# slatedb/slatedb

Hardware: AMD Instinct MI355X
Metric: GiB/s device-resident SST block encode+bloom, 64 MiB sorted KV, 1/2/4/8 GPU (higher is better)
Workload: dtype u8

## Files before the change

slatedb_amd/csrc/sdb_encode.h:

```cpp
#pragma once
#include <hip/hip_runtime.h>
#include <stdint.h>

#include "../../include/slatedb_amd.h"
#include "sdb_workspace.h"

namespace sdb {

constexpr uint32_t kChunk = 2048;
constexpr uint32_t kResolveLds = 96 * 1024;
#ifndef SDB_EMIT_CRC_MFMA
#define SDB_EMIT_CRC_SLICE
#endif
#ifdef SDB_EMIT_CRC_SLICE
constexpr uint32_t kCrcLds = 36 * 1024;
#else
constexpr uint32_t kCrcLds = 56 * 1024;
#endif
constexpr uint32_t kImgCap = 4096 + 64;
constexpr uint32_t kStageCap = 4096;
constexpr uint32_t kStageGuard = 64;
constexpr uint32_t kKeyStageCap = 1024;
constexpr uint32_t kPieceRowMax = 4000, kPieceKeyMax = 960, kPieceValMax = 3968;
constexpr uint32_t kSegLook = 1024;
constexpr uint32_t kSegSpan = kChunk + kSegLook;
constexpr uint32_t kSegThreads = 512;
constexpr uint32_t kFactsThreads = 1024;
constexpr uint32_t kFactsPerT = 2;
constexpr uint32_t kFactsEntries = kFactsThreads * kFactsPerT;
constexpr uint32_t kSegLds = (2 * kSegSpan + 4) * 4 + kChunk * 6;
constexpr uint32_t kSegLdsMax = 64 * 1024;
constexpr uint32_t kHashPerT = kChunk / kSegThreads;
#ifndef SDB_EMIT_WAVES
#define SDB_EMIT_WAVES 16
#endif
constexpr uint32_t kEmitThreads = 64 * SDB_EMIT_WAVES;
constexpr uint32_t kEmitWgPerCu = 1;
constexpr uint32_t kEmitWaveLds = kStageGuard + kImgCap + 16 + kKeyStageCap + 64 * 16;
constexpr uint32_t kEmitLds = kCrcLds + 16 + (kEmitThreads / 64) * kEmitWaveLds;
constexpr uint32_t kEnumLds = kChunk * 16 + 11 * kChunk * 2;
constexpr uint32_t kEnumTabLds = 11 * kChunk * 2;
constexpr uint32_t kGroupThreads = 1024;
constexpr uint32_t kEnumThreads = 512;
constexpr uint32_t kGroupLds = kResolveLds;

struct BloomPlan {
    uint32_t k, m;
    uint32_t sb;
    uint32_t nslices, T, tiles;
    uint32_t one_pass;
    uint32_t pad;
    uint64_t mmod;
};
struct BloomSlots {
    uint32_t *count;
    uint32_t *slot;
    uint32_t cap;
};

struct BlockDesc {
    uint32_t s, e;
    uint64_t off;
    uint64_t vs, ve, ks, ke;
    uint32_t bb, pad;
};

struct EncodeArgs {
    const uint8_t *key_bytes;
    const uint64_t *key_off;
    const uint8_t *val_bytes;
    const uint64_t *val_off;
    const uint8_t *kind;
    const uint64_t *seq;
    const int64_t *create_ts;
    const int64_t *expire_ts;
    const uint8_t *ts_mask;
    uint64_t n;
    uint32_t block_size;
    uint32_t restart_interval;
    uint32_t version;
    uint32_t wal;
    uint32_t nchunks;
    uint32_t seg_look;
    uint32_t *lcp;
    uint32_t *szr, *sznr;
    uint32_t nfacts;
    uint32_t *row_scratch;
    uint32_t *next;
    uint32_t *bbytes;
    uint32_t *tab_exit;
    uint32_t *tab_cnt;
    uint64_t *tab_bytes;
    uint32_t *anchor_e;
    uint32_t *anchor_blk;
    uint64_t *anchor_byte;
    unsigned long long *err;
    uint32_t *wmax;
    uint32_t *slow_count;
    uint32_t *slow_list;
    uint32_t *big_count;
    uint32_t *big_list;
    BlockDesc *desc;
    uint64_t *stat_part;
    uint32_t *huge_part;
    uint32_t *wmax_part;
    unsigned long long *err_part;
    uint32_t *gtab_exit;
    uint32_t *gtab_cnt;
    uint64_t *gtab_bytes;
    uint32_t *mode;
    uint32_t group;
    uint32_t bloom_fused;
    BloomPlan bpl;
    BloomSlots bq;
    uint8_t *bloom_out;
    uint32_t *done;
    uint32_t nprep_wg;
    uint32_t seg_lds;
    uint8_t *out_data;
    uint64_t *out_block_off;
    uint32_t *out_block_first;
    uint32_t *out_index_key_len;
// ... 175 lines not shown
```

slatedb_amd/csrc/sdb_encode.hip:

```cpp
#include <stdlib.h>

#include <atomic>
#include <mutex>

#include "sdb_bloom.h"
#include "sdb_crc.h"
#include "sdb_crc_mfma.h"

namespace sdb {

#ifndef SDB_SEG_WAVES
#define SDB_SEG_WAVES 8
#endif
#ifdef SDB_PHASE_TIMING
__device__ uint64_t g_phase[1024][8];
#define PHASE_MARK(i)                                                              \
    do {                                                                           \
        __syncthreads();                                                           \
        if (threadIdx.x == 0 && blockIdx.x < 1024) g_phase[blockIdx.x][i] = __builtin_amdgcn_s_memtime(); \
    } while (0)
__device__ uint64_t g_wave_phase[8192][8];
__device__ uint64_t g_phase_enum[1024][8];
#define PHASE_MARK_E(i)                                                                  \
    do {                                                                                 \
// ... 274 lines not shown
#ifdef SDB_EXP_FACTS_NOBIN
        bloom_bin_core<kFactsPerT>(blockIdx.x, hh, dd, 0, a.bpl, a.bq, blds);
#else
        bloom_bin_core<kFactsPerT>(blockIdx.x, hh, dd, nk, a.bpl, a.bq, blds);
#endif
    }
}

SDB_DEV uint32_t walk_size_v2(const EncodeArgs &a, uint64_t j, bool rs) {
    EntryFacts f = entry_facts(a, j);
    return rs ? f.s_r : f.s_nr;
}

SDB_DEV void seg_chunk(const EncodeArgs &a, uint8_t *smem, uint32_t k) {
    uint32_t *s_P = (uint32_t *)smem;
    uint32_t *s_R = s_P + kSegSpan + 4;
    uint32_t *s_bb = s_R + kSegSpan;
    uint16_t *s_nx = (uint16_t *)(s_bb + kChunk);
    __shared__ uint32_t s_len[kSegThreads / 64];
    const uint32_t tid = threadIdx.x, nt = blockDim.x;
    const uint64_t cs = (uint64_t)k * kChunk;
    const uint64_t ce = cs + kChunk < a.n ? cs + kChunk : a.n;
    const uint64_t se = ce + a.seg_look < a.n ? ce + a.seg_look : a.n;
    const uint32_t cn = (uint32_t)(ce - cs), sn = (uint32_t)(se - cs);
    const uint64_t bs = a.block_size;
    const uint32_t clampv = (uint32_t)(bs + 16);
    const bool v2 = a.version == 2 && bs <= (1u << 20);
    const uint32_t ri = a.restart_interval;
    PHASE_MARK(0);
    constexpr uint32_t kPerT = kSegSpan / kSegThreads;
    const uint32_t lane = (uint32_t)lane_id();
    uint32_t zr[kPerT], znr[kPerT];
#pragma unroll
    for (uint32_t u = 0; u < kPerT; u++) {
        const uint32_t x = tid + u * nt;
        zr[u] = znr[u] = 0;
        if (x < sn) {
            zr[u] = a.szr[cs + x];
            znr[u] = a.sznr[cs + x];
        }
    }
#pragma unroll
    for (uint32_t u = 0; u < kPerT; u++) {
        const uint32_t x = tid + u * nt;
        if (x >= sn) continue;
        if (v2) {
            const uint32_t cr = zr[u] < clampv ? zr[u] : clampv, cnr = znr[u] < clampv ? znr[u] : clampv;
            s_P[x] = cnr;
            s_R[x] = cr + 2 - cnr;
        }
    }
    __syncthreads();
    PHASE_MARK(1);
    if (v2) {
        __shared__ uint32_t s_wt[kPerT * (kSegThreads / 64) + 1];
        const uint32_t wv = tid >> 6;
        uint32_t v[kPerT], inc[kPerT];
#pragma unroll
        for (uint32_t u = 0; u < kPerT; u++) {
            const uint32_t x = tid + u * nt;
            v[u] = x < sn ? s_P[x] : 0;
            inc[u] = wave_incl_scan(v[u]);
            if (lane == 63) s_wt[u * (nt >> 6) + wv] = inc[u];
        }
        __syncthreads();
        if (tid < 64) {
            const uint32_t nw = kPerT * (nt >> 6);
            const uint32_t t = tid < nw ? s_wt[tid] : 0, it = wave_incl_scan(t);
            __builtin_amdgcn_wave_barrier();
            if (tid < nw) s_wt[tid] = it - t;
            if (tid == 63) s_P[sn] = it;
        }
        __syncthreads();
#pragma unroll
        for (uint32_t u = 0; u < kPerT; u++) {
            const uint32_t x = tid + u * nt;
            if (x < sn) s_P[x] = s_wt[u * (nt >> 6) + wv] + inc[u] - v[u];
        }
        PHASE_MARK(2);
    }
    __syncthreads();
    PHASE_MARK(3);
    uint32_t maxlen = 0;
    for (uint32_t x = tid; x < cn; x += nt) {
        const uint64_t b = cs + x;
        uint64_t j;
        uint64_t bytes;
        if (v2) {
            const uint32_t Pb = s_P[x];
            auto size_of = [&](uint32_t e) -> uint64_t {
                uint64_t sz = 2ull + (s_P[e] - Pb);
                for (uint32_t r = x; r < e; r += ri) sz += s_R[r];
                return sz;
            };
            uint32_t lo = x + 1;
            uint32_t e = lo;
            {
                const uint32_t w = (x + 64 < sn ? x + 64 : sn) - x;
                const uint32_t mean = (s_P[x + w] - Pb) / w + 1;
                uint32_t est = x + (uint32_t)(bs / mean);
                e = est < lo ? lo : (est > sn ? sn : est);
            }
            if (size_of(e) <= bs) {
                while (e < sn && size_of(e + 1) <= bs) e++;
            } else {
                while (e > lo && size_of(e) > bs) e--;
            }
            j = cs + e;
            if (e == lo) bytes = 2ull + a.szr[b] + 2;
            else bytes = size_of(e);
            if (e == sn && se < a.n) {
                uint64_t acc = bytes;
                uint32_t p = e - x, ph = p % ri;
                while (j < a.n) {
                    const bool rs = ph == 0;
                    const uint64_t add = (uint64_t)walk_size_v2(a, j, rs) + (rs ? 2 : 0);
                    if (acc + add > bs) break;
                    acc += add;
                    j++;
                    if (++ph == ri) ph = 0;
                }
                bytes = acc;
            }
        } else if (a.version == 2) {
            uint64_t acc = 2;
            j = b;
            uint32_t p = 0, ph = 0;
            while (j < a.n) {
                const bool rs = ph == 0;
                const uint64_t add = (uint64_t)walk_size_v2(a, j, rs) + (rs ? 2 : 0);
                if (p > 0 && acc + add > bs) break;
                acc += add;
                j++;
                p++;
                if (++ph == ri) ph = 0;
            }
            bytes = acc;
        } else {
            uint64_t acc = 2;
            j = b;
            uint32_t p = 0;
            const uint64_t fko = a.key_off[b];
            const uint32_t fkl = (uint32_t)(a.key_off[b + 1] - fko);
            while (j < a.n) {
                uint32_t prefix = 0;
                if (p > 0) {
                    uint64_t ko = a.key_off[j];
                    prefix = lcp_bytes(a.key_bytes + fko, fkl, a.key_bytes + ko, (uint32_t)(a.key_off[j + 1] - ko));
                }
                uint64_t sr = a.szr[j];
                uint64_t sz = sr - prefix;
                if (p > 0 && acc + sz > bs) break;
                acc += sz + 2;
                j++;
                p++;
            }
            bytes = acc;
        }
        const uint32_t bb = (uint32_t)(bytes + 4);
        a.next[b] = (uint32_t)j;
        a.bbytes[b] = bb;
        s_bb[x] = bb;
        const uint64_t rel = j - cs;
        s_nx[x] = (uint16_t)(rel < 0xFFFF ? rel : 0xFFFF);
        const uint32_t len = (uint32_t)(j - b);
        maxlen = len > maxlen ? len : maxlen;
    }
    maxlen = wave_max(maxlen);
    if (lane_id() == 0) s_len[tid >> 6] = maxlen;
    __syncthreads();
    if (tid == 0) {
        uint32_t m = 0;
        for (uint32_t q = 0; q < nt / 64; q++) m = s_len[q] > m ? s_len[q] : m;
        a.wmax_part[k] = m;
    }
    PHASE_MARK(4);
    __shared__ uint32_t s_wc;
    if (tid == 0) {
        uint32_t wc = a.seg_look;
        if (v2) {
            uint32_t lo = 0, hi = sn;
            while (lo < hi) {
                const uint32_t mid = (lo + hi + 1) >> 1;
                if ((uint64_t)(s_P[mid] - s_P[0]) + 2 <= bs) lo = mid;
                else hi = mid - 1;
            }
            wc = lo + 1 < wc ? lo + 1 : wc;
        }
        s_wc = wc;
    }
    __syncthreads();
    const uint32_t Wc = s_wc;
    uint32_t *j_nx = s_P;
    uint64_t *j_bb = (uint64_t *)(s_P + kChunk);
    static_assert(3 * kChunk <= 2 * kSegSpan + 4, "jump tables alias s_P / s_R");
    constexpr uint32_t kJU = kChunk / kSegThreads;
    {
        uint32_t jn[kJU];
        uint64_t jb[kJU];
#pragma unroll
        for (uint32_t u = 0; u < kJU; u++) {
            const uint32_t x = tid + u * nt;
            jn[u] = 0;
            jb[u] = 0;
            if (x < cn) {
                const uint32_t n1 = s_nx[x];
                uint64_t b = s_bb[x];
                uint32_t n = n1, c = 1;
                if (n1 < cn) {
                    b += s_bb[n1];
                    n = s_nx[n1];
                    c = 2;
                }
                jn[u] = n | c << 16;
                jb[u] = b;
            }
        }
#pragma unroll
        for (uint32_t u = 0; u < kJU; u++) {
            const uint32_t x = tid + u * nt;
            if (x < cn) {
                j_nx[x] = jn[u];
                j_bb[x] = jb[u];
            }
        }
        __syncthreads();
#pragma unroll
        for (uint32_t u = 0; u < kJU; u++) {
            const uint32_t x = tid + u * nt;
            if (x < cn) {
                const uint32_t n = jn[u] & 0xFFFF;
                if (n < cn) {
                    const uint32_t w = j_nx[n];
                    jb[u] += j_bb[n];
                    jn[u] = (w & 0xFFFF) | ((jn[u] >> 16) + (w >> 16)) << 16;
                }
            }
        }
        __syncthreads();
#pragma unroll
        for (uint32_t u = 0; u < kJU; u++) {
            const uint32_t x = tid + u * nt;
            if (x < cn) {
                j_nx[x] = jn[u];
                j_bb[x] = jb[u];
            }
        }
        __syncthreads();
    }
    for (uint32_t c = tid; c < Wc; c += nt) {
        uint32_t e = c, cnt = 0;
        uint64_t by = 0;
        while (e < cn) {
            const uint32_t v = j_nx[e];
            by += j_bb[e];
            cnt += v >> 16;
            e = v & 0xFFFF;
        }
        const uint64_t t = (uint64_t)k * a.seg_look + c;
        a.tab_exit[t] = c >= cn ? (uint32_t)ce : (e == 0xFFFF ? 0xFFFFFFFFu : (uint32_t)(cs + e));
        a.tab_cnt[t] = cnt;
        a.tab_bytes[t] = by;
    }
    PHASE_MARK(5);
    PHASE_MARK(6);
}

__global__ __launch_bounds__(kSegThreads, SDB_SEG_WAVES) void k_seg(SstSet P) {
    const EncodeArgs a = make_args(P, blockIdx.y);
    extern __shared__ __attribute__((aligned(16))) uint8_t smem[];
    if (blockIdx.x < P.max_chunks) {
        if (blockIdx.x < a.nchunks) seg_chunk(a, smem, blockIdx.x);
    } else if (a.bloom_fused && blockIdx.x - P.max_chunks < a.bpl.nslices) {
        bloom_fill_slice(blockIdx.x - P.max_chunks, a.key_bytes, a.key_off, a.n, a.bpl, a.bq, a.bloom_out,
                         a.bloom_len, (uint32_t *)smem);
    }
}

__global__ __launch_bounds__(kGroupThreads) void k_group(SstSet P) {
// ... 1555 lines not shown
            } else {
                q = (int)(r + l);
            }
            if (q >= 0) {
                if (tr_lds) {
                    tr[2 * q] = (uint8_t)(br >> 8);
                    tr[2 * q + 1] = (uint8_t)br;
                } else {
                    gblk[D + 2 * q] = (uint8_t)(br >> 8);
                    gblk[D + 2 * q + 1] = (uint8_t)br;
                }
            }
        }
        wave_sync();
        if (l < 16) ((lu32 *)(img - kStageGuard))[l] = 0;
        if (r == 0 && l == 0) ((lu32 *)img)[0] = ~((const lu32 *)img)[0];
        wave_sync();
        crc = crc_shift_bytes(crc, Lp) ^ wave_crc_image_ra(img, Lp) ^ 0xFFFFFFFFu;
        uint8_t *gp = gblk + base;
        const uint32_t nfull = Lp >> 4;
        for (uint32_t cc = l; cc < nfull; cc += 64) {
            u32x4 v = ((const lu128 *)img)[cc];
            if (cc == 0 && r == 0) v.x = ~v.x;
            __builtin_memcpy(gp + 16 * cc, &v, 16);
        }
        if (l < (Lp & 15)) {
            const uint32_t x = (nfull << 4) + l;
            gp[x] = (r == 0 && x < 4) ? (uint8_t)~img[x] : img[x];
        }
        pu += (uint32_t)__popcll(__ballot(prow && kind == SDB_KIND_VALUE));
        de += (uint32_t)__popcll(__ballot(prow && kind == SDB_KIND_TOMBSTONE));
        me += (uint32_t)__popcll(__ballot(prow && kind == SDB_KIND_MERGE));
        base += Lp;
        r += c;
        wave_sync();
    }
    if (base != D && l == 0) report_error(a.err, d.s, SDB_DEVICE_ERROR);
    if (tr_lds) {
        if (l == 0) {
            tr[2 * noffs] = (uint8_t)(noffs >> 8);
            tr[2 * noffs + 1] = (uint8_t)noffs;
        }
        wave_sync();
        const uint8_t v = l < Tl ? tr[l] : 0;
        if (l < 16) ((lu32 *)(img - kStageGuard))[l] = 0;
        img[l] = v;
        wave_sync();
        crc = crc_shift_bytes(crc, Tl) ^ wave_crc_image_ra(img, Tl) ^ 0xFFFFFFFFu;
        if (l < Tl) gblk[D + l] = v;
    } else {
        if (l == 0) {
            gblk[D + 2 * noffs] = (uint8_t)(noffs >> 8);
            gblk[D + 2 * noffs + 1] = (uint8_t)noffs;
        }
        __threadfence_block();
        wave_sync();
    }
    for (uint32_t t = tr_lds ? Lc : D; t < Lc; t += 4096) {
        const uint32_t w = Lc - t < 4096 ? Lc - t : 4096;
        for (uint32_t q = l; q < w; q += 64) img[q] = gblk[t + q];
        if (l < 16) ((lu32 *)(img - kStageGuard))[l] = 0;
        for (uint32_t q = w + l; q < ((w + 63) & ~63u); q += 64) img[q] = 0;
        wave_sync();
        crc = crc_shift_bytes(crc, w) ^ wave_crc_image_ra(img, w) ^ 0xFFFFFFFFu;
        wave_sync();
    }
    crc ^= 0xFFFFFFFFu;
    if (l == 0) {
        gblk[Lc] = (uint8_t)(crc >> 24);
        gblk[Lc + 1] = (uint8_t)(crc >> 16);
        gblk[Lc + 2] = (uint8_t)(crc >> 8);
        gblk[Lc + 3] = (uint8_t)crc;
        a.out_block_stats[3 * (uint64_t)blk] = (uint16_t)pu;
        a.out_block_stats[3 * (uint64_t)blk + 1] = (uint16_t)de;
        a.out_block_stats[3 * (uint64_t)blk + 2] = (uint16_t)me;
        a.out_index_key_len[blk] = ik;
    }
    wave_sync();
}

template <int V>
SDB_DEV void emit_slow_blocks(const EncodeArgs &a, uint8_t *scratch, const uint32_t (*s_crc)[256]);

SDB_DEV void finish_summary(const EncodeArgs &a) {
    sdb_sst_summary *s = a.summary;
    const unsigned long long e = atomicOr(a.err, 0ull);
    s->max_block_entries = *a.wmax;
    uint64_t bl = a.bloom_len;
    if (a.bloom_len_dev) {
        bl = *a.bloom_len_dev;
        if (bl == ~0ull) {
            bl = 0;
            if (e == ~0ull) {
                s->status = SDB_INVALID_ARGUMENT;
                s->first_error_entry = 0;
            }
        }
    }
    s->bloom_len = bl;
    s->num_probes = a.num_probes;
    s->filter_built = a.filter_built;
    if (e != ~0ull) {
        s->status = (int32_t)(e & 0xFF);
        s->first_error_entry = e >> 8;
    }
}

template <int V>
__global__ __launch_bounds__(kEmitThreads, 1) void k_emit(SstSet P) {
    extern __shared__ __attribute__((aligned(16))) uint8_t smem[];
#ifdef SDB_PHASE_TIMING
    const uint64_t rt0 = __builtin_amdgcn_s_memrealtime(), mt0 = __builtin_amdgcn_s_memtime();
#endif
    const uint32_t wave = (uint32_t)__builtin_amdgcn_readfirstlane((int)(threadIdx.x >> 6)), wpb = blockDim.x >> 6;
    const uint32_t gw = blockIdx.x * wpb + wave;
    (void)gw;
    const uint32_t l = (uint32_t)lane_id();
    uint64_t ph[8] = {0, 0, 0, 0, 0, 0, 0, 0};
    uint32_t nbl = 0;
    if (l < P.count) {
        const EncodeArgs ai = make_args(P, l);
        if (*ai.err == ~0ull) nbl = ai.anchor_blk[ai.nchunks];
    }
    const uint32_t vpre = wave_incl_scan(nbl);
    const uint32_t nb = (uint32_t)__builtin_amdgcn_readlane((int)vpre, kMaxSsts - 1);
    bool run = nb > 0;
    if (lds_addr((const void *)smem) != 0) {
        if (threadIdx.x == 0)
            for (uint32_t i = 0; i < P.count; i++) report_error(make_args(P, i).err, 0, SDB_DEVICE_ERROR);
        run = false;
    }
    auto locate = [&](uint32_t g, uint32_t &si, uint32_t &lb) {
        const uint64_t m = __ballot(l + 1 < kMaxSsts && vpre <= g && vpre < nb);
        si = (uint32_t)__popcll(m);
        lb = g - (si ? (uint32_t)__builtin_amdgcn_readlane((int)vpre, (int)si - 1) : 0u);
    };
    auto desc_lanes = [&](uint32_t g, uint32_t r1) -> uint32_t {
        uint32_t si, lb;
        locate(g < r1 ? g : r1 - 1, si, lb);
        return ((const uint32_t *)make_args(P, si).desc)[14 * (uint64_t)lb + (l < 14 ? l : 13)];
    };
    if (run) {
        lu32 *crc = (lu32 *)smem;
        (void)crc;
        const uint32_t r0 = (uint32_t)((uint64_t)nb * blockIdx.x / gridDim.x);
        const uint32_t r1 = (uint32_t)((uint64_t)nb * (blockIdx.x + 1) / gridDim.x);
        uint32_t blk = r0 + wave;
        const bool any = blk < r1;
        uint32_t dvc = any ? desc_lanes(blk, r1) : 0u;
#ifdef SDB_EMIT_CRC_SLICE
        crc_tables_to_lds(crc);
#else
        crc_mfma_tables_to_lds(crc);
#endif
        EmitData pd;
        EmitMeta mc;
        bool fc = false;
        if (any) {
            uint32_t si, lb;
            locate(blk, si, lb);
            const BlockDesc d0 = desc_from_lanes(dvc);
            fc = emit_fast(d0);
            emit_prefetch_data(make_args(P, si), desc_or_empty(d0, fc), pd);
            emit_prefetch_meta(make_args(P, si), desc_or_empty(d0, fc), mc);
        }
        __syncthreads();
        for (uint32_t i = 0; i < P.count; i++) {
            const EncodeArgs ai = make_args(P, i);
            if (*ai.err == ~0ull && *ai.slow_count)
#ifdef SDB_EMIT_CRC_SLICE
                emit_slow_blocks<V>(ai, (uint8_t *)smem + kCrcLds + 16, (const uint32_t(*)[256])smem);
#else
                emit_slow_blocks<V>(ai, (uint8_t *)smem + kCrcLds + 16, (const uint32_t(*)[256])c_crc.t);
#endif
        }
        __syncthreads();
        if (threadIdx.x == 0) *(lu32 *)(smem + kCrcLds) = blockDim.x >> 6;
        __syncthreads();
        lu8 *wbase = (lu8 *)smem + kCrcLds + 16 + wave * kEmitWaveLds;
        lu8 *img = wbase + kStageGuard;
        lu8 *kst = img + kImgCap + 16;
        lSpanCopy *rtab = (lSpanCopy *)(kst + kKeyStageCap);
        lu32 *ticket = (lu32 *)(smem + kCrcLds);
        auto take = [&]() -> uint32_t {
            uint32_t t = 0;
            if (l == 0) t = __hip_atomic_fetch_add(ticket, 1u, __ATOMIC_RELAXED, __HIP_MEMORY_SCOPE_WORKGROUP);
            return r0 + (uint32_t)__builtin_amdgcn_readfirstlane((int)t);
        };
        if (any) {
            uint32_t nblk = take();
            uint32_t dvn = desc_lanes(nblk, r1);
            __builtin_amdgcn_s_waitcnt(0x0F70);
            while (true) {
                emit_stage(desc_or_empty(desc_from_lanes(dvc), fc), pd, img, kst);
                const bool more = nblk < r1;
                uint32_t si, lb;
                locate(more ? nblk : r1 - 1, si, lb);
                const BlockDesc dn0 = desc_from_lanes(dvn);
                const bool fn = more && emit_fast(dn0);
                const BlockDesc dn = desc_or_empty(dn0, fn);
                emit_prefetch_data(make_args(P, si), dn, pd);
                EmitMeta mn;
                emit_prefetch_meta(make_args(P, si), dn, mn);
                const uint32_t n2 = take();
                const uint32_t dv2 = desc_lanes(n2, r1);
                uint32_t csi, clb;
                locate(blk, csi, clb);
                emit_block<V>(make_args(P, csi), clb, desc_or_empty(desc_from_lanes(dvc), fc), fc, mc, img, kst, rtab, crc, ph);
                if (!more) break;
                blk = nblk;
                nblk = n2;
                dvc = dvn;
                dvn = dv2;
                mc = mn;
                fc = fn;
            }
        }
    }
#ifdef SDB_PHASE_TIMING
    if (lane_id() == 0 && gw < 8192)
        for (int i = 0; i < 8; i++) g_wave_phase[gw][i] = ph[i];
    const uint64_t rt1 = __builtin_amdgcn_s_memrealtime(), mt1 = __builtin_amdgcn_s_memtime();
    if (lane_id() == 0 && gw < 8192) {
        g_wave_rt[gw][0] = rt0;
        g_wave_rt[gw][1] = rt1;
        g_wave_rt[gw][2] = mt0;
        g_wave_rt[gw][3] = mt1;
    }
#endif
    __syncthreads();
    if (threadIdx.x == 0) {
        __threadfence();
        if (atomicAdd(&make_args(P, 0).done[0], 1u) == gridDim.x - 1) {
            __threadfence();
            for (uint32_t i = 0; i < P.count; i++) finish_summary(make_args(P, i));
        }
    }
}

template <int V>
SDB_DEV void emit_slow_blocks(const EncodeArgs &a, uint8_t *scratch, const uint32_t (*s_crc)[256]) {
    uint8_t *s_win = scratch;
    uint64_t *s_size = (uint64_t *)(scratch + 8192);
    uint64_t *s_off = (uint64_t *)(scratch + 8192 + 8 * kEmitThreads);
    const uint32_t nslow = *a.slow_count;
    for (uint32_t it = blockIdx.x; it < nslow; it += gridDim.x) {
        const uint32_t blk = a.slow_list[it];
        const uint64_t b = a.out_block_first[blk];
        const uint64_t e = a.next[b];
        const uint64_t off = a.out_block_off[blk];
        const uint32_t ne = (uint32_t)(e - b);
        uint8_t *dst = a.out_data + off;
        const uint32_t ri = a.restart_interval;
        const uint64_t fko = a.key_off[b];
        const uint32_t fkl = (uint32_t)(a.key_off[b + 1] - fko);
        uint64_t D = 0;
        for (uint32_t i0 = 0; i0 < ne; i0 += blockDim.x) {
            uint32_t i = i0 + threadIdx.x;
            RowInfo r;
            uint64_t seq = 0;
            int64_t ets = 0, cts = 0;
            if (i < ne) {
                uint64_t j = b + i;
                uint64_t ko = a.key_off[j];
                uint32_t klen = (uint32_t)(a.key_off[j + 1] - ko);
                uint8_t kd = a.kind ? a.kind[j] : 0;
                uint8_t m = a.ts_mask ? a.ts_mask[j] : 0;
                uint32_t vlen = kd == SDB_KIND_TOMBSTONE ? 0 : (uint32_t)(a.val_off[j + 1] - a.val_off[j]);
                uint32_t shared;
                if (V == 2) shared = (i % ri == 0) ? 0 : a.lcp[j];
                else shared = (i == 0) ? 0 : lcp_bytes(a.key_bytes + fko, fkl, a.key_bytes + ko, klen);
                r.shared = shared;
                r.suf = klen - shared;
                r.vlen = vlen;
                r.key_src = ko + shared;
                r.val_src = a.val_off[j];
                r.flags = (uint8_t)((kd == SDB_KIND_MERGE ? SDB_FLAG_MERGE_OPERAND : 0) |
                                    (kd == SDB_KIND_TOMBSTONE ? SDB_FLAG_TOMBSTONE : 0) |
                                    ((m & SDB_TS_EXPIRE) ? SDB_FLAG_HAS_EXPIRE_TS : 0) |
                                    ((m & SDB_TS_CREATE) ? SDB_FLAG_HAS_CREATE_TS : 0));
                const uint32_t ts8 = 8u * (((m & SDB_TS_CREATE) != 0) + ((m & SDB_TS_EXPIRE) != 0));
                if (V == 2) r.size = varint_len(shared) + varint_len(r.suf) + varint_len(vlen) + r.suf + vlen + 9 + ts8;
                else r.size = 4 + r.suf + 9 + ts8 + (kd == SDB_KIND_TOMBSTONE ? 0 : 4 + vlen);
                seq = a.seq ? a.seq[j] : 0;
                ets = (m & SDB_TS_EXPIRE) ? a.expire_ts[j] : 0;
                cts = (m & SDB_TS_CREATE) ? a.create_ts[j] : 0;
                s_size[threadIdx.x] = r.size;
            } else {
// ... 31 lines not shown
        __threadfence();
        __syncthreads();
        if (threadIdx.x == 0) {
            uint32_t pu = 0, de = 0, me = 0;
            for (uint64_t j = b; j < e; j++) {
                uint8_t kd = a.kind ? a.kind[j] : 0;
                pu += kd == SDB_KIND_VALUE;
                de += kd == SDB_KIND_TOMBSTONE;
                me += kd == SDB_KIND_MERGE;
            }
            a.out_block_stats[3 * (uint64_t)blk] = (uint16_t)pu;
            a.out_block_stats[3 * (uint64_t)blk + 1] = (uint16_t)de;
            a.out_block_stats[3 * (uint64_t)blk + 2] = (uint16_t)me;
            uint32_t ik = 0;
            if (b > 0 && !a.wal) {
                uint64_t fl = a.key_off[b + 1] - a.key_off[b];
                uint64_t pl = a.key_off[b] - a.key_off[b - 1];
                uint32_t lc = a.lcp[b];
                ik = (lc == pl && pl == fl) ? (uint32_t)fl : lc + 1;
            }
            a.out_index_key_len[blk] = ik;
        }
        uint32_t noffs = (V == 2) ? (ne + ri - 1) / ri : ne;
        for (uint32_t q = threadIdx.x; q < noffs; q += blockDim.x) {
            uint32_t ro = a.row_scratch[b + (V == 2 ? (uint64_t)q * ri : q)];
            dst[D + 2 * q] = (uint8_t)(ro >> 8);
            dst[D + 2 * q + 1] = (uint8_t)ro;
        }
        if (threadIdx.x == 0) {
            dst[D + 2 * noffs] = (uint8_t)(noffs >> 8);
            dst[D + 2 * noffs + 1] = (uint8_t)noffs;
        }
        __threadfence();
        __syncthreads();
        const uint64_t Lc = D + 2 * (uint64_t)noffs + 2;
        if (threadIdx.x < 64) {
            uint64_t nwin = (Lc + 4095) >> 12;
            uint64_t first = Lc - ((nwin - 1) << 12);
            uint32_t acc = 0;
            for (uint64_t w = 0; w < nwin; w++) {
                uint64_t wbeg = (w == 0) ? 0 : first + ((w - 1) << 12);
                uint32_t wlen = (uint32_t)((w == 0) ? first : 4096);
                for (uint32_t q = threadIdx.x; q < wlen; q += 64)
                    s_win[16 + q] = dst[wbeg + q] ^ (wbeg + q < 4 ? 0xFF : 0);
                wave_sync();
                uint32_t raw = wave_crc_raw_lds(s_win + 16, wlen, (const uint32_t(*)[256])s_crc, false);
                acc = (w == 0) ? raw : (gf_mul(c_shift.window, acc) ^ raw);
                wave_sync();
            }
            uint32_t crc = acc ^ 0xFFFFFFFFu;
            if (threadIdx.x == 0) {
                dst[Lc] = (uint8_t)(crc >> 24);
                dst[Lc + 1] = (uint8_t)(crc >> 16);
                dst[Lc + 2] = (uint8_t)(crc >> 8);
                dst[Lc + 3] = (uint8_t)crc;
            }
        }
        __syncthreads();
    }
}

template __global__ void k_emit<1>(SstSet);
template __global__ void k_emit<2>(SstSet);

template <int V>
__global__ __launch_bounds__(kEmitThreads, 1) void k_emit_big(SstSet P) {
    extern __shared__ __attribute__((aligned(16))) uint8_t smem[];
    uint32_t pre[kMaxSsts + 1];
    pre[0] = 0;
#pragma unroll
    for (uint32_t i = 0; i < kMaxSsts; i++) {
        uint32_t nb = 0;
        if (i < P.count) {
            const EncodeArgs ai = make_args(P, i);
            if (*ai.err == ~0ull) nb = *ai.big_count;
        }
        pre[i + 1] = pre[i] + nb;
    }
    const uint32_t total = pre[kMaxSsts];
    if (!total || lds_addr((const void *)smem) != 0) return;
    crc_tables_to_lds((lu32 *)smem);
    __syncthreads();
    const uint32_t wave = (uint32_t)__builtin_amdgcn_readfirstlane((int)(threadIdx.x >> 6)), wpb = blockDim.x >> 6;
    lu8 *img = (lu8 *)smem + kCrcLds + 16 + wave * kEmitWaveLds + kStageGuard;
    lu8 *kst = img + kImgCap + 16;
    lSpanCopy *rtab = (lSpanCopy *)(kst + kKeyStageCap);
    for (uint32_t g = blockIdx.x * wpb + wave; g < total; g += gridDim.x * wpb) {
        uint32_t si = 0, base = 0;
#pragma unroll
        for (uint32_t j = 1; j < kMaxSsts; j++)
            if (g >= pre[j] && pre[j] < total) {
                si = j;
                base = pre[j];
            }
        const EncodeArgs a = make_args(P, si);
        const uint32_t blk = a.big_list[g - base];
        emit_big<V>(a, blk, a.desc[blk], img, kst, rtab);
    }
}
template __global__ void k_emit_big<1>(SstSet);
template __global__ void k_emit_big<2>(SstSet);

__global__ void k_init_summary(EncodeArgs a) {
    if (threadIdx.x == 0) {
        sdb_sst_summary *s = a.summary;
        s->data_len = 0;
        s->num_blocks = 0;
        s->num_entries = a.n;
        s->raw_key_size = 0;
        s->raw_val_size = 0;
        s->num_puts = s->num_deletes = s->num_merges = 0;
        s->bloom_len = 0;
        s->num_probes = 0;
        s->filter_built = 0;
        s->status = 0;
        s->max_block_entries = 0;
        s->first_error_entry = ~0ull;
        *a.err = ~0ull;
        *a.wmax = 0;
        *a.slow_count = 0;
        *a.big_count = 0;
        if (a.n == 0 && a.block_cap + 1 > 0) {
            a.out_block_off[0] = 0;
            a.out_block_first[0] = 0;
        }
    }
}

__global__ void k_finish_summary(EncodeArgs a, uint64_t bloom_len, uint32_t num_probes, uint32_t built) {
    if (threadIdx.x == 0) {
        sdb_sst_summary *s = a.summary;
        unsigned long long e = *a.err;
        s->max_block_entries = *a.wmax;
        s->bloom_len = bloom_len;
        s->num_probes = num_probes;
        s->filter_built = built;
        if (e != ~0ull) {
            s->status = (int32_t)(e & 0xFF);
            s->first_error_entry = e >> 8;
        }
    }
}

#ifdef SDB_PHASE_TIMING
extern "C" int sdb_diag_wave_phase(uint64_t *out, int nwaves) {
    return hipMemcpyFromSymbol(out, HIP_SYMBOL(g_wave_phase), sizeof(uint64_t) * 8 * nwaves) == hipSuccess ? 0 : -1;
}
extern "C" int sdb_diag_wave_rt(uint64_t *out, int nwaves) {
#ifdef SDB_PHASE_TIMING
    return hipMemcpyFromSymbol(out, HIP_SYMBOL(g_wave_rt), sizeof(uint64_t) * 4 * nwaves) == hipSuccess ? 0 : -1;
#else
    return -1;
#endif
}
extern "C" int sdb_diag_enum_phase(uint64_t *out, int nblocks) {
    return hipMemcpyFromSymbol(out, HIP_SYMBOL(g_phase_enum), sizeof(uint64_t) * 8 * nblocks) == hipSuccess ? 0 : -1;
}
extern "C" int sdb_diag_phase_times(uint64_t *out, int nblocks) {
    return hipMemcpyFromSymbol(out, HIP_SYMBOL(g_phase), sizeof(uint64_t) * 8 * nblocks) == hipSuccess ? 0 : -1;
}
#endif

static int g_cus = 0;
static uint32_t g_emit_threads = kEmitThreads, g_emit_wg_per_cu = kEmitWgPerCu;
static std::once_flag g_attrs_once;
static uint32_t g_emit_grid = 0;
constexpr int kMaxDevices = 64;
static std::atomic<uint32_t> g_builders[kMaxDevices];
static int current_device() {
    int dev = 0;
    return hipGetDevice(&dev) == hipSuccess && dev >= 0 && dev < kMaxDevices ? dev : 0;
}
static uint32_t emit_grid() {
    if (g_emit_grid) return g_emit_grid;
    const uint32_t full = (uint32_t)(g_cus > 0 ? g_emit_wg_per_cu * g_cus : 512);
    const uint32_t b = g_builders[current_device()].load(std::memory_order_relaxed);
    return b > 1 ? (full / b ? full / b : 1u) : full;
}
static uint32_t emit_lds() { return kCrcLds + 16 + (g_emit_threads / 64) * kEmitWaveLds; }
static void set_lds_attrs() {
    std::call_once(g_attrs_once, [] {
        int dev = 0;
        (void)hipGetDevice(&dev);
        (void)hipDeviceGetAttribute(&g_cus, hipDeviceAttributeMultiprocessorCount, dev);
        if (const char *e = getenv("SDB_EMIT_THREADS")) {
            uint32_t t = (uint32_t)atoi(e);
            if (t >= 64 && t <= kEmitThreads && t % 64 == 0) g_emit_threads = t;
        }
        if (const char *e = getenv("SDB_EMIT_GRID")) {
            const int t = atoi(e);
            if (t >= 1 && t <= 4096) g_emit_grid = (uint32_t)t;
        }
        if (const char *e = getenv("SDB_EMIT_WG_PER_CU")) {
            uint32_t t = (uint32_t)atoi(e);
            if (t >= 1 && t <= 32) g_emit_wg_per_cu = t;
        }
        (void)hipFuncSetAttribute((const void *)k_emit<1>, hipFuncAttributeMaxDynamicSharedMemorySize, (int)kEmitLds);
        (void)hipFuncSetAttribute((const void *)k_emit<2>, hipFuncAttributeMaxDynamicSharedMemorySize, (int)kEmitLds);
        (void)hipFuncSetAttribute((const void *)k_emit_big<1>, hipFuncAttributeMaxDynamicSharedMemorySize, (int)kEmitLds);
        (void)hipFuncSetAttribute((const void *)k_emit_big<2>, hipFuncAttributeMaxDynamicSharedMemorySize, (int)kEmitLds);
        (void)hipFuncSetAttribute((const void *)k_enum, hipFuncAttributeMaxDynamicSharedMemorySize, (int)kEnumLds);
        (void)hipFuncSetAttribute((const void *)k_group, hipFuncAttributeMaxDynamicSharedMemorySize, (int)kGroupLds);
        (void)hipFuncSetAttribute((const void *)k_anchor, hipFuncAttributeMaxDynamicSharedMemorySize, (int)kAnchorLds);
        (void)hipFuncSetAttribute((const void *)k_seg, hipFuncAttributeMaxDynamicSharedMemorySize, 96 * 1024);
        (void)hipFuncSetAttribute((const void *)k_facts, hipFuncAttributeMaxDynamicSharedMemorySize, (int)kBinLds);
        (void)hipGetLastError();
    });
}

static_assert(kChunk == kFactsEntries && kFactsThreads == kBinThreads, "bloom tiles are k_facts' chunks of kChunk keys");

hipError_t launch_encode_set(const SstSet &P, size_t bin_lds, size_t fill_lds, hipStream_t st) {
    set_lds_attrs();
    if (!P.count) return hipSuccess;
    stage_mark(st, kStFacts, true);
    hipLaunchKernelGGL(k_facts, dim3(P.max_facts, P.count), dim3(kFactsThreads), P.max_tiles ? bin_lds : 0, st, P);
    stage_mark(st, kStFacts, false);
    stage_mark(st, kStSeg, true);
    const size_t seg_lds = kSegLds > fill_lds ? kSegLds : fill_lds;
    hipLaunchKernelGGL(k_seg, dim3(P.max_chunks + P.max_slices, P.count), dim3(kSegThreads), seg_lds, st, P);
    stage_mark(st, kStSeg, false);
    stage_mark(st, kStAnchor, true);
    hipLaunchKernelGGL(k_anchor, dim3(1, P.count), dim3(kAnchorThreads), kAnchorLds, st, P);
    stage_mark(st, kStAnchor, false);
    stage_mark(st, kStBlocks, true);
    hipLaunchKernelGGL(k_blocks, dim3(P.max_chunks, P.count), dim3(kBlkThreads), 0, st, P);
    stage_mark(st, kStBlocks, false);
    stage_mark(st, kStEmitBig, true);
    const uint32_t big_grid = P.block_size > 4096 ? emit_grid() : (emit_grid() < 32 ? emit_grid() : 32);
    if (P.version == 2) hipLaunchKernelGGL(k_emit_big<2>, dim3(big_grid), dim3(g_emit_threads), emit_lds(), st, P);
    else hipLaunchKernelGGL(k_emit_big<1>, dim3(big_grid), dim3(g_emit_threads), emit_lds(), st, P);
    stage_mark(st, kStEmitBig, false);
    stage_mark(st, kStEmit, true);
    if (P.version == 2) hipLaunchKernelGGL(k_emit<2>, dim3(emit_grid()), dim3(g_emit_threads), emit_lds(), st, P);
    else hipLaunchKernelGGL(k_emit<1>, dim3(emit_grid()), dim3(g_emit_threads), emit_lds(), st, P);
    stage_mark(st, kStEmit, false);
    return hipGetLastError();
}

hipError_t launch_encode_prep(const SstSet &P, hipStream_t st) {
    set_lds_attrs();
    if (!P.count) return hipSuccess;
    hipLaunchKernelGGL(k_facts, dim3(P.max_facts, P.count), dim3(kFactsThreads), 0, st, P);
    hipLaunchKernelGGL(k_seg, dim3(P.max_chunks, P.count), dim3(kSegThreads), kSegLds, st, P);
    hipLaunchKernelGGL(k_group, dim3(P.max_groups, P.count), dim3(kGroupThreads), kGroupLds, st, P);
    return hipGetLastError();
}

hipError_t launch_encode_empty(EncodeArgs a, hipStream_t st) {
    hipLaunchKernelGGL(k_init_summary, dim3(1), dim3(64), 0, st, a);
    hipLaunchKernelGGL(k_finish_summary, dim3(1), dim3(64), 0, st, a, a.bloom_len, a.num_probes, a.filter_built);
    return hipGetLastError();
}

}

extern "C" sdb_status sdb_set_concurrent_builders(uint32_t builders) {
    if (builders == 0) return SDB_INVALID_ARGUMENT;
    sdb::g_builders[sdb::current_device()].store(builders, std::memory_order_relaxed);
    return SDB_OK;
}
```

Measured before the change: 1256.

## Replace static per-workgroup block ranges in k_emit with global batched work queue

The emit kernel previously split blocks into fixed contiguous ranges per workgroup and handed them out to waves through a workgroup-local ticket. Now each workgroup claims batches of 16 blocks from a device-wide atomic counter, with a small LDS ring that prefetches the next batch starts. Waves still take tickets locally and map them to batch offsets. The goal is dynamic load balancing across CUs when block costs vary, at the price of global atomics, a spin-wait on the ring, and use of a done[1] slot as the queue counter, which has to be zeroed before launch.

```diff
diff --git a/slatedb_amd/csrc/sdb_encode.h b/slatedb_amd/csrc/sdb_encode.h
--- a/slatedb_amd/csrc/sdb_encode.h
+++ b/slatedb_amd/csrc/sdb_encode.h
@@ -37,7 +37,13 @@
 constexpr uint32_t kEmitThreads = 64 * SDB_EMIT_WAVES;
 constexpr uint32_t kEmitWgPerCu = 1;
 constexpr uint32_t kEmitWaveLds = kStageGuard + kImgCap + 16 + kKeyStageCap + 64 * 16;
-constexpr uint32_t kEmitLds = kCrcLds + 16 + (kEmitThreads / 64) * kEmitWaveLds;
+#ifndef SDB_EMIT_BATCH
+#define SDB_EMIT_BATCH 16
+#endif
+constexpr uint32_t kEmitBatch = SDB_EMIT_BATCH;
+static_assert((kEmitBatch & (kEmitBatch - 1)) == 0 && kEmitBatch >= kEmitThreads / 64, "k_emit batch");
+constexpr uint32_t kEmitCtlLds = 48;
+constexpr uint32_t kEmitLds = kCrcLds + kEmitCtlLds + (kEmitThreads / 64) * kEmitWaveLds;
 constexpr uint32_t kEnumLds = kChunk * 16 + 11 * kChunk * 2;
 constexpr uint32_t kEnumTabLds = 11 * kChunk * 2;
 constexpr uint32_t kGroupThreads = 1024;
diff --git a/slatedb_amd/csrc/sdb_encode.hip b/slatedb_amd/csrc/sdb_encode.hip
--- a/slatedb_amd/csrc/sdb_encode.hip
+++ b/slatedb_amd/csrc/sdb_encode.hip
@@ -2214,6 +2214,19 @@
 template <int V>
 SDB_DEV void emit_slow_blocks(const EncodeArgs &a, uint8_t *scratch, const uint32_t (*s_crc)[256]);
 
+typedef __attribute__((address_space(3))) uint64_t lu64;
+SDB_DEV void ring_put(lu64 *ring, uint32_t q, uint32_t first) {
+    __hip_atomic_store(ring + (q & 3), (uint64_t)q << 32 | first, __ATOMIC_RELAXED, __HIP_MEMORY_SCOPE_WORKGROUP);
+}
+SDB_DEV uint32_t ring_get(lu64 *ring, uint32_t q) {
+    uint64_t s = __hip_atomic_load(ring + (q & 3), __ATOMIC_RELAXED, __HIP_MEMORY_SCOPE_WORKGROUP);
+    while ((int32_t)((uint32_t)(s >> 32) - q) < 0) {
+        __builtin_amdgcn_s_sleep(1);
+        s = __hip_atomic_load(ring + (q & 3), __ATOMIC_RELAXED, __HIP_MEMORY_SCOPE_WORKGROUP);
+    }
+    return (uint32_t)s;
+}
+
 SDB_DEV void finish_summary(const EncodeArgs &a) {
     sdb_sst_summary *s = a.summary;
     const unsigned long long e = atomicOr(a.err, 0ull);
@@ -2267,19 +2280,28 @@
         si = (uint32_t)__popcll(m);
         lb = g - (si ? (uint32_t)__builtin_amdgcn_readlane((int)vpre, (int)si - 1) : 0u);
     };
-    auto desc_lanes = [&](uint32_t g, uint32_t r1) -> uint32_t {
+    auto desc_lanes = [&](uint32_t g) -> uint32_t {
         uint32_t si, lb;
-        locate(g < r1 ? g : r1 - 1, si, lb);
+        locate(g < nb ? g : nb - 1, si, lb);
         return ((const uint32_t *)make_args(P, si).desc)[14 * (uint64_t)lb + (l < 14 ? l : 13)];
+    };
+    auto batch_first = [&](uint32_t c) -> uint32_t {
+        const uint64_t f = (uint64_t)c * kEmitBatch;
+        return f < nb ? (uint32_t)f : nb;
     };
     if (run) {
         lu32 *crc = (lu32 *)smem;
         (void)crc;
-        const uint32_t r0 = (uint32_t)((uint64_t)nb * blockIdx.x / gridDim.x);
-        const uint32_t r1 = (uint32_t)((uint64_t)nb * (blockIdx.x + 1) / gridDim.x);
-        uint32_t blk = r0 + wave;
-        const bool any = blk < r1;
-        uint32_t dvc = any ? desc_lanes(blk, r1) : 0u;
+        lu32 *ticket = (lu32 *)(smem + kCrcLds);
+        lu64 *ring = (lu64 *)(smem + kCrcLds + 16);
+        uint32_t *queue = &make_args(P, 0).done[1];
+        const uint32_t f0 = batch_first(blockIdx.x);
+        uint32_t blk = f0 + wave;
+        const bool any = blk < nb;
+        uint32_t c1 = 0;
+        if (threadIdx.x == 0 && f0 < nb)
+            c1 = __hip_atomic_fetch_add(queue, 2u, __ATOMIC_RELAXED, __HIP_MEMORY_SCOPE_AGENT) + gridDim.x;
+        uint32_t dvc = any ? desc_lanes(blk) : 0u;
 #ifdef SDB_EMIT_CRC_SLICE
         crc_tables_to_lds(crc);
 #else
@@ -2301,33 +2323,49 @@
             const EncodeArgs ai = make_args(P, i);
             if (*ai.err == ~0ull && *ai.slow_count)
 #ifdef SDB_EMIT_CRC_SLICE
-                emit_slow_blocks<V>(ai, (uint8_t *)smem + kCrcLds + 16, (const uint32_t(*)[256])smem);
+                emit_slow_blocks<V>(ai, (uint8_t *)smem + kCrcLds + kEmitCtlLds, (const uint32_t(*)[256])smem);
 #else
-                emit_slow_blocks<V>(ai, (uint8_t *)smem + kCrcLds + 16, (const uint32_t(*)[256])c_crc.t);
+                emit_slow_blocks<V>(ai, (uint8_t *)smem + kCrcLds + kEmitCtlLds, (const uint32_t(*)[256])c_crc.t);
 #endif
         }
         __syncthreads();
-        if (threadIdx.x == 0) *(lu32 *)(smem + kCrcLds) = blockDim.x >> 6;
+        if (threadIdx.x == 0) {
+            *ticket = wpb;
+            ring_put(ring, 0, f0);
+            ring_put(ring, 1, f0 < nb ? batch_first(c1) : nb);
+            ring_put(ring, 2, f0 < nb ? batch_first(c1 + 1) : nb);
+            ring_put(ring, 3u - 4u, nb);
+        }
         __syncthreads();
-        lu8 *wbase = (lu8 *)smem + kCrcLds + 16 + wave * kEmitWaveLds;
+        lu8 *wbase = (lu8 *)smem + kCrcLds + kEmitCtlLds + wave * kEmitWaveLds;
         lu8 *img = wbase + kStageGuard;
         lu8 *kst = img + kImgCap + 16;
         lSpanCopy *rtab = (lSpanCopy *)(kst + kKeyStageCap);
-        lu32 *ticket = (lu32 *)(smem + kCrcLds);
         auto take = [&]() -> uint32_t {
-            uint32_t t = 0;
-            if (l == 0) t = __hip_atomic_fetch_add(ticket, 1u, __ATOMIC_RELAXED, __HIP_MEMORY_SCOPE_WORKGROUP);
-            return r0 + (uint32_t)__builtin_amdgcn_readfirstlane((int)t);
+            uint32_t g = 0;
+            if (l == 0) {
+                const uint32_t p = __hip_atomic_fetch_add(ticket, 1u, __ATOMIC_RELAXED, __HIP_MEMORY_SCOPE_WORKGROUP);
+                const uint32_t q = p / kEmitBatch;
+                const uint32_t f = ring_get(ring, q);
+                if (p % kEmitBatch == 0) {
+                    uint32_t fn = nb;
+                    if (f < nb)
+                        fn = batch_first(__hip_atomic_fetch_add(queue, 1u, __ATOMIC_RELAXED, __HIP_MEMORY_SCOPE_AGENT) + gridDim.x);
+                    ring_put(ring, q + 2, fn);
+                }
+                g = f + p % kEmitBatch;
+            }
+            return (uint32_t)__builtin_amdgcn_readfirstlane((int)g);
         };
         if (any) {
             uint32_t nblk = take();
-            uint32_t dvn = desc_lanes(nblk, r1);
+            uint32_t dvn = desc_lanes(nblk);
             __builtin_amdgcn_s_waitcnt(0x0F70);
             while (true) {
                 emit_stage(desc_or_empty(desc_from_lanes(dvc), fc), pd, img, kst);
-                const bool more = nblk < r1;
+                const bool more = nblk < nb;
                 uint32_t si, lb;
-                locate(more ? nblk : r1 - 1, si, lb);
+                locate(more ? nblk : nb - 1, si, lb);
                 const BlockDesc dn0 = desc_from_lanes(dvn);
                 const bool fn = more && emit_fast(dn0);
                 const BlockDesc dn = desc_or_empty(dn0, fn);
@@ -2335,7 +2373,7 @@
                 EmitMeta mn;
                 emit_prefetch_meta(make_args(P, si), dn, mn);
                 const uint32_t n2 = take();
-                const uint32_t dv2 = desc_lanes(n2, r1);
+                const uint32_t dv2 = desc_lanes(n2);
                 uint32_t csi, clb;
                 locate(blk, csi, clb);
                 emit_block<V>(make_args(P, csi), clb, desc_or_empty(desc_from_lanes(dvc), fc), fc, mc, img, kst, rtab, crc, ph);
@@ -2533,7 +2571,7 @@
     crc_tables_to_lds((lu32 *)smem);
     __syncthreads();
     const uint32_t wave = (uint32_t)__builtin_amdgcn_readfirstlane((int)(threadIdx.x >> 6)), wpb = blockDim.x >> 6;
-    lu8 *img = (lu8 *)smem + kCrcLds + 16 + wave * kEmitWaveLds + kStageGuard;
+    lu8 *img = (lu8 *)smem + kCrcLds + kEmitCtlLds + wave * kEmitWaveLds + kStageGuard;
     lu8 *kst = img + kImgCap + 16;
     lSpanCopy *rtab = (lSpanCopy *)(kst + kKeyStageCap);
     for (uint32_t g = blockIdx.x * wpb + wave; g < total; g += gridDim.x * wpb) {
@@ -2628,7 +2666,7 @@
     const uint32_t b = g_builders[current_device()].load(std::memory_order_relaxed);
     return b > 1 ? (full / b ? full / b : 1u) : full;
 }
-static uint32_t emit_lds() { return kCrcLds + 16 + (g_emit_threads / 64) * kEmitWaveLds; }
+static uint32_t emit_lds() { return kCrcLds + kEmitCtlLds + (g_emit_threads / 64) * kEmitWaveLds; }
 static void set_lds_attrs() {
     std::call_once(g_attrs_once, [] {
         int dev = 0;
```

Result: slower. 1240 (-1.3%).

## Scan v2 block boundaries incrementally per thread and skip slow-block sync in emit

Applied to the files above, without the earlier changes.

Each thread now owns four consecutive chunk entries. The block-end search runs incrementally, reusing the previous entry's end and restart-sum instead of recomputing size_of from scratch. Results are written as 16-byte vector stores, and the division estimate is replaced by a float reciprocal. In k_emit, SSTs with pending slow blocks are found once through a ballot, and the extra barriers are skipped when there are none. The risks are changed block boundaries from the float estimate (it is only a starting hint) and partitioning that is less balanced than the strided loop.

```diff
diff --git a/slatedb_amd/csrc/sdb_encode.hip b/slatedb_amd/csrc/sdb_encode.hip
--- a/slatedb_amd/csrc/sdb_encode.hip
+++ b/slatedb_amd/csrc/sdb_encode.hip
@@ -380,39 +380,58 @@
     __syncthreads();
     PHASE_MARK(3);
     uint32_t maxlen = 0;
-    for (uint32_t x = tid; x < cn; x += nt) {
-        const uint64_t b = cs + x;
-        uint64_t j;
-        uint64_t bytes;
-        if (v2) {
+    constexpr uint32_t kJU = kChunk / kSegThreads;
+    static_assert(kJU == 4, "a thread's next() / block bytes are stored as one 16-byte vector");
+    if (v2) {
+        const uint32_t x0 = tid * kJU;
+        uint4 vj = {0, 0, 0, 0}, vb = {0, 0, 0, 0};
+        uint32_t e = 0;
+#pragma unroll 1
+        for (uint32_t u = 0; u < kJU && x0 + u < cn; u++) {
+            const uint32_t x = x0 + u, lo = x + 1;
+            const uint64_t b = cs + x;
             const uint32_t Pb = s_P[x];
-            auto size_of = [&](uint32_t e) -> uint64_t {
-                uint64_t sz = 2ull + (s_P[e] - Pb);
-                for (uint32_t r = x; r < e; r += ri) sz += s_R[r];
-                return sz;
-            };
-            uint32_t lo = x + 1;
-            uint32_t e = lo;
-            {
-                const uint32_t w = (x + 64 < sn ? x + 64 : sn) - x;
-                const uint32_t mean = (s_P[x + w] - Pb) / w + 1;
-                uint32_t est = x + (uint32_t)(bs / mean);
+            if (u == 0) {
+                const uint32_t w = (x + 64 < sn ? x + 64 : sn) - x, d = s_P[x + w] - Pb;
+                const uint32_t mean = (w == 64 ? d >> 6 : d / w) + 1;
+                const uint32_t est = x + (uint32_t)((float)bs * __builtin_amdgcn_rcpf((float)mean));
                 e = est < lo ? lo : (est > sn ? sn : est);
-            }
-            if (size_of(e) <= bs) {
-                while (e < sn && size_of(e + 1) <= bs) e++;
             } else {
-                while (e > lo && size_of(e) > bs) e--;
-            }
-            j = cs + e;
-            if (e == lo) bytes = 2ull + a.szr[b] + 2;
-            else bytes = size_of(e);
+                e = e < lo ? lo : e;
+            }
+            uint64_t rs = 0;
+            uint32_t nr = x;
+            for (; nr < e; nr += ri) rs += s_R[nr];
+            uint64_t sz = 2ull + (s_P[e] - Pb) + rs;
+            if (sz <= bs) {
+                while (e < sn) {
+                    const uint64_t add = e == nr ? s_R[e] : 0;
+                    const uint64_t s1 = 2ull + (s_P[e + 1] - Pb) + rs + add;
+                    if (s1 > bs) break;
+                    sz = s1;
+                    rs += add;
+                    if (e == nr) nr += ri;
+                    e++;
+                }
+            } else {
+                while (e > lo) {
+                    e--;
+                    if (e + ri == nr) {
+                        nr = e;
+                        rs -= s_R[e];
+                    }
+                    sz = 2ull + (s_P[e] - Pb) + rs;
+                    if (sz <= bs) break;
+                }
+            }
+            uint64_t j = cs + e;
+            uint64_t bytes = e == lo ? 2ull + a.szr[b] + 2 : sz;
             if (e == sn && se < a.n) {
                 uint64_t acc = bytes;
                 uint32_t p = e - x, ph = p % ri;
                 while (j < a.n) {
-                    const bool rs = ph == 0;
-                    const uint64_t add = (uint64_t)walk_size_v2(a, j, rs) + (rs ? 2 : 0);
+                    const bool rst = ph == 0;
+                    const uint64_t add = (uint64_t)walk_size_v2(a, j, rst) + (rst ? 2 : 0);
                     if (acc + add > bs) break;
                     acc += add;
                     j++;
@@ -420,7 +439,44 @@
                 }
                 bytes = acc;
             }
-        } else if (a.version == 2) {
+            const uint32_t bb = (uint32_t)(bytes + 4);
+            vj.x = u == 0 ? (uint32_t)j : vj.x;
+            vj.y = u == 1 ? (uint32_t)j : vj.y;
+            vj.z = u == 2 ? (uint32_t)j : vj.z;
+            vj.w = u == 3 ? (uint32_t)j : vj.w;
+            vb.x = u == 0 ? bb : vb.x;
+            vb.y = u == 1 ? bb : vb.y;
+            vb.z = u == 2 ? bb : vb.z;
+            vb.w = u == 3 ? bb : vb.w;
+            const uint32_t len = (uint32_t)(j - b);
+            maxlen = len > maxlen ? len : maxlen;
+        }
+        auto rel16 = [&](uint32_t j) -> uint32_t {
+            const uint32_t rel = j - (uint32_t)cs;
+            return rel < 0xFFFF ? rel : 0xFFFF;
+        };
+        if (x0 + kJU <= cn) {
+            *(uint4 *)(a.next + cs + x0) = vj;
+            *(uint4 *)(a.bbytes + cs + x0) = vb;
+            *(uint4 *)(s_bb + x0) = vb;
+            *(uint2 *)(s_nx + x0) = make_uint2(rel16(vj.x) | rel16(vj.y) << 16, rel16(vj.z) | rel16(vj.w) << 16);
+        } else if (x0 < cn) {
+            const uint32_t tj[kJU] = {vj.x, vj.y, vj.z, vj.w}, tb[kJU] = {vb.x, vb.y, vb.z, vb.w};
+#pragma unroll
+            for (uint32_t u = 0; u < kJU; u++)
+                if (x0 + u < cn) {
+                    a.next[cs + x0 + u] = tj[u];
+                    a.bbytes[cs + x0 + u] = tb[u];
+                    s_bb[x0 + u] = tb[u];
+                    s_nx[x0 + u] = (uint16_t)rel16(tj[u]);
+                }
+        }
+    }
+    for (uint32_t x = tid; !v2 && x < cn; x += nt) {
+        const uint64_t b = cs + x;
+        uint64_t j;
+        uint64_t bytes;
+        if (a.version == 2) {
             uint64_t acc = 2;
             j = b;
             uint32_t p = 0, ph = 0;
@@ -492,7 +548,6 @@
     uint32_t *j_nx = s_P;
     uint64_t *j_bb = (uint64_t *)(s_P + kChunk);
     static_assert(3 * kChunk <= 2 * kSegSpan + 4, "jump tables alias s_P / s_R");
-    constexpr uint32_t kJU = kChunk / kSegThreads;
     {
         uint32_t jn[kJU];
         uint64_t jb[kJU];
@@ -2250,10 +2305,17 @@
     const uint32_t l = (uint32_t)lane_id();
     uint64_t ph[8] = {0, 0, 0, 0, 0, 0, 0, 0};
     uint32_t nbl = 0;
+    bool has_slow = false;
     if (l < P.count) {
         const EncodeArgs ai = make_args(P, l);
-        if (*ai.err == ~0ull) nbl = ai.anchor_blk[ai.nchunks];
-    }
+        const unsigned long long er = *ai.err;
+        const uint32_t ab = ai.anchor_blk[ai.nchunks], sc = *ai.slow_count;
+        if (er == ~0ull) {
+            nbl = ab;
+            has_slow = sc != 0;
+        }
+    }
+    const uint32_t slow_w = (uint32_t)__ballot(has_slow);
     const uint32_t vpre = wave_incl_scan(nbl);
     const uint32_t nb = (uint32_t)__builtin_amdgcn_readlane((int)vpre, kMaxSsts - 1);
     bool run = nb > 0;
@@ -2296,19 +2358,23 @@
             emit_prefetch_data(make_args(P, si), desc_or_empty(d0, fc), pd);
             emit_prefetch_meta(make_args(P, si), desc_or_empty(d0, fc), mc);
         }
+        if (threadIdx.x == 0) {
+            *(lu32 *)(smem + kCrcLds) = blockDim.x >> 6;
+            *(lu32 *)(smem + kCrcLds + 4) = slow_w;
+        }
         __syncthreads();
-        for (uint32_t i = 0; i < P.count; i++) {
-            const EncodeArgs ai = make_args(P, i);
-            if (*ai.err == ~0ull && *ai.slow_count)
+        const uint32_t slow = (uint32_t)__builtin_amdgcn_readfirstlane((int)*(lu32 *)(smem + kCrcLds + 4));
+        if (slow) {
+            for (uint32_t m = slow; m; m &= m - 1) {
+                const EncodeArgs ai = make_args(P, (uint32_t)__builtin_ctz(m));
 #ifdef SDB_EMIT_CRC_SLICE
                 emit_slow_blocks<V>(ai, (uint8_t *)smem + kCrcLds + 16, (const uint32_t(*)[256])smem);
 #else
                 emit_slow_blocks<V>(ai, (uint8_t *)smem + kCrcLds + 16, (const uint32_t(*)[256])c_crc.t);
 #endif
-        }
-        __syncthreads();
-        if (threadIdx.x == 0) *(lu32 *)(smem + kCrcLds) = blockDim.x >> 6;
-        __syncthreads();
+            }
+            __syncthreads();
+        }
         lu8 *wbase = (lu8 *)smem + kCrcLds + 16 + wave * kEmitWaveLds;
         lu8 *img = wbase + kStageGuard;
         lu8 *kst = img + kImgCap + 16;
```

After: 1226 before, 1239 after, median of 6. 1.01x the previous value.
